# Fabstir/fabstir-vectordb

Measured on AMD Instinct MI355X. Metric: k-NN queries/sec at recall@10>=0.95, 1Mx384 f32, higher is better.
Workload: dtype f32

## Files before the change

### fabstir-vectordb_amd/csrc/fvdb_hip.cpp

```cpp
#include "fvdb_internal.h"

#include <unistd.h>

#include <algorithm>
#include <atomic>
#include <cmath>
#include <condition_variable>
#include <mutex>
#include <cstdio>
#include <cstdlib>
#include <cstring>
#include <map>
#include <new>
#include <string>
#include <vector>

#include "common.h"
#include "kernels_misc.h"
#include "kernels_scan.h"
#include "kernels_coarse.h"
#include "kernels_mfma.h"
#include "kernels_mfma_wg.h"
#include "kernels_util.h"
#include "kernels_maint.h"
// ... 115 lines not shown
  SC_STATS = 4,
};
constexpr size_t kScalarsBytes = 64;

struct IvfScratch {
  std::mutex enq;
  bool pend_filter = false;
  bool pending_profile = false, pend_coarse = false, pend_fine = false, collecting = false;
  std::vector<DBuf*> bufs;
  struct Buf : DBuf {
    explicit Buf(IvfScratch* set) { set->bufs.push_back(this); }
  };
  Buf s_qnorm{this}, s_A{this};
  Buf s_qh{this}, s_qn2{this}, s_thr{this}, s_tA{this}, s_pa{this}, s_surv{this}, s_scnt{this}, s_fail{this}, s_mslots{this};
  Buf s_sdist{this}, s_probes2{this};
  Buf s_q{this}, s_cpart{this}, s_probes{this}, s_cnt{this}, s_fill{this}, s_eoff{this}, s_ioff{this}, s_entries{this};
  Buf s_part{this}, s_scalars{this}, s_ceoff{this}, s_cioff{this};
  Buf s_in{this}, s_slots{this}, s_ids{this}, s_clusters{this}, s_out_ids{this}, s_out_dist{this}, s_out_cnt{this}, s_cdist{this};
  hipEvent_t sev[EV_COUNT] = {};
  uint32_t* scalar(ScalWord w) const { return s_scalars.as<uint32_t>() + w; }
  void release_all() {
    for (DBuf* b : bufs) b->release();
    for (auto& e : sev) {
      if (e) (void)hipEventDestroy(e);
      e = nullptr;
    }
  }
};

struct fvdb_ivf : IvfScratch {
  static constexpr uint32_t kSlots = 16;
// ... 70 lines not shown
  static bool has(const char* name) { return getenv(name) != nullptr; }
  static int tiles(int m) { return m >= 4 ? 4 : (m >= 2 ? 2 : 1); }
  bool coarse_exact = has("FVDB_COARSE_EXACT");
  bool scan_exact = has("FVDB_SCAN_EXACT");
  uint32_t scan_wgs_per_cu = (uint32_t)num("FVDB_SCAN_WGS_PER_CU", 8);
  int segb = num("FVDB_SEGB", 0);
  bool no_shared_thr = has("FVDB_NO_SHARED_THR");
  int mfma_m = tiles(num("FVDB_MFMA_M", 2));
  int mfma_segb = num("FVDB_MFMA_SEGB", 0);
  uint32_t mfma_wgs_per_cu = (uint32_t)std::max(1, num("FVDB_MFMA_WGS_PER_CU", 2));
  bool mfma_groups_in_item = num("FVDB_MFMA_GROUPS_IN_ITEM", 0) != 0;
  bool mfma_wg = num("FVDB_MFMA_WG", 1) != 0;
  int mfma_wg_m = num("FVDB_MFMA_WG_M", 4) >= 4 ? 4 : 2;
  uint32_t mfma_wg_segb = (uint32_t)std::max(4, num("FVDB_MFMA_WG_SEGB", 16));
  uint32_t mfma_wg_per_cu = (uint32_t)std::max(1, num("FVDB_MFMA_WG_PER_CU", 2));
  int mfma_wg_tail_pct = num("FVDB_MFMA_WG_TAIL_PCT", 25);
  int mfma_wg_segb_tail = num("FVDB_MFMA_WG_SEGB_TAIL", 4);
  uint32_t mfma_cap_a = (uint32_t)std::max(1, num("FVDB_MFMA_CAP_A", 4));
  bool mfma_threshold_pass = has("FVDB_MFMA_THRESHOLD_PASS");
  uint32_t mfma_segb_a = (uint32_t)std::max(1, num("FVDB_MFMA_SEGB_A", 1));
  bool mfma_no_refine = has("FVDB_MFMA_NO_REFINE");
#ifdef FVDB_MFMA_STAMPS_BUILD
  int mfma_stamps = num("FVDB_MFMA_STAMPS", 0);
#endif
};
const IvfKnobs& ivf_knobs() {
  static const IvfKnobs knobs{};
  return knobs;
}

struct ScanLaunch {
// ... 192 lines not shown
  if (max_blocks >= 4096) return 16;
  if (pairs >= 4096) return 4;
  if (pairs >= 512) return 2;
  return 1;
}
uint32_t pick_segb(fvdb_ivf* ivf, uint32_t B, uint32_t nprobe) {
  const int forced = ivf_knobs().segb;
  return forced > 0 ? (uint32_t)forced : segb_for(ivf->max_list_blocks, B, nprobe);
}
uint64_t queries_per_gib(uint32_t max_blocks, uint32_t segb, uint32_t k, uint32_t np) {
  const uint64_t per_q = (uint64_t)np * std::max<uint32_t>(1, cdiv(max_blocks, segb)) * k * 8;
  return (1ull << 30) / std::max<uint64_t>(per_q, 1);
}

void launch_plan(fvdb_ivf* ivf, const Env& E, const uint32_t* probes, uint32_t n, uint32_t np, uint32_t segb, uint32_t Q,
                 unsigned long long* stats, uint32_t* rezero_cnt, uint32_t lsplit = 0xFFFFFFFFu, uint32_t segb_tail = 0) {
  fvdb_ctx* ctx = E.ctx;
  IvfScratch& S = *E.S;
  const uint32_t* list_off = ivf->t_off.as<uint32_t>();
  hipLaunchKernelGGL(plan_count_kernel, dim3(cdiv(n, 256)), dim3(256), 0, ctx->stream, probes, n, S.s_cnt.as<uint32_t>(),
                     list_off);
  hipLaunchKernelGGL(plan_scan_kernel, dim3(1), dim3(1024), 0, ctx->stream, S.s_cnt.as<uint32_t>(), list_off,
                     ivf->t_len.as<uint32_t>(), ivf->nlist, segb, Q, S.s_eoff.as<uint32_t>(), S.s_ioff.as<uint32_t>(),
                     S.s_fill.as<uint32_t>(), S.scalar(SC_FINE_ITEMS), S.scalar(SC_FINE_HEAD), stats, rezero_cnt, lsplit,
                     segb_tail);
  hipLaunchKernelGGL(plan_fill_kernel, dim3(cdiv(n, 256)), dim3(256), 0, ctx->stream, probes, n, np,
                     S.s_eoff.as<uint32_t>(), S.s_fill.as<uint32_t>(), S.s_entries.as<uint2>(), list_off);
}
inline unsigned long long* scan_stats(const IvfScratch& S) { return (unsigned long long*)S.scalar(SC_STATS); }

int plan_scratch(fvdb_ivf* ivf, const Env& E, uint32_t B, uint32_t np) {
  fvdb_ctx* ctx = E.ctx;
  IvfScratch& S = *E.S;
  const uint32_t nlist = ivf->nlist;
  HIPCHK(ctx, S.s_cnt.ensure((size_t)nlist * 4));
  HIPCHK(ctx, S.s_fill.ensure((size_t)nlist * 4));
  HIPCHK(ctx, S.s_eoff.ensure((size_t)(nlist + 1) * 4));
  HIPCHK(ctx, S.s_ioff.ensure((size_t)(nlist + 1) * 4));
  HIPCHK(ctx, S.s_entries.ensure((size_t)B * np * 8));
  return FVDB_OK;
// ... 29 lines not shown

constexpr uint32_t kMfmaSlack = 6;
constexpr uint32_t kMfmaCmax = 4096;

bool mfma_shape_ok(const fvdb_ivf* ivf, uint32_t B, uint32_t k, uint32_t np) {
  return ivf->dpad % 16 == 0 && k + kMfmaSlack <= 32 && np <= 256 && B >= 32 && B <= 16384;
}
inline bool half_rows(const fvdb_ivf* ivf) { return ivf->f16 || ivf->pool.half != nullptr; }
inline int x_rounded(const fvdb_ivf* ivf) { return ivf->f16 ? 0 : (ivf->pool.half ? 1 : 2); }

struct MfmaPlan {
  bool wg;
  int M;
  uint32_t Q, ka, cmax;
  uint32_t segb, segbA;
  uint32_t lsplit, segb_tail;
  uint32_t fsegb, fmaxsegs;
  uint64_t fpart;
  uint32_t grid, wg_grid, wg_lds;
  bool half_rows;
  int x_rounded;
};

int mfma_plan(fvdb_ivf* ivf, fvdb_ctx* ctx, const IvfKnobs& kn, uint32_t B, uint32_t k, uint32_t np, MfmaPlan* out) {
  MfmaPlan P{};
  P.half_rows = half_rows(ivf);
  P.x_rounded = x_rounded(ivf);
  int wgM = kn.mfma_wg_m;
  if (mfma_wg_lds_bytes(ivf->dpad, 16u * wgM) > 64u * 1024u) wgM = 2;
  P.wg = kn.mfma_wg && kn.mfma_m == 2 && P.half_rows && ivf->dpad % 128 == 0 &&
         mfma_wg_lds_bytes(ivf->dpad, 16u * wgM) <= 64u * 1024u;
  P.M = P.wg ? wgM : kn.mfma_m;
  P.Q = 16u * P.M;
  P.ka = k + kMfmaSlack;
  P.cmax = kMfmaCmax;
  P.segbA = kn.mfma_segb_a;
  P.segb = P.wg ? kn.mfma_wg_segb : (kn.mfma_segb > 0 ? (uint32_t)kn.mfma_segb : pick_segb(ivf, B, np));
  P.lsplit = 0xFFFFFFFFu;
  P.segb_tail = P.segb;
  if (P.wg && kn.mfma_wg_tail_pct > 0 && kn.mfma_wg_segb_tail > 0 && (uint32_t)kn.mfma_wg_segb_tail < P.segb) {
    P.lsplit = (uint32_t)((uint64_t)ivf->nlist * (uint32_t)(100 - std::min(kn.mfma_wg_tail_pct, 100)) / 100);
    P.segb_tail = (uint32_t)kn.mfma_wg_segb_tail;
  }
  P.fsegb = pick_segb(ivf, B, np);
  P.fmaxsegs = std::max<uint32_t>(1, cdiv(ivf->max_list_blocks, P.fsegb));
  P.fpart = (uint64_t)B * np * P.fmaxsegs * k;
  if (P.fpart >= (1ull << 32)) FAIL(ctx, FVDB_E_UNSUPPORTED, "batch too large for one launch (sub-batch it)");
  P.grid = (uint32_t)ctx->num_cus * kn.mfma_wgs_per_cu;
  P.wg_grid = (uint32_t)ctx->num_cus * kn.mfma_wg_per_cu;
  P.wg_lds = mfma_wg_lds_bytes(ivf->dpad, P.Q);
  *out = P;
  return FVDB_OK;
}

int mfma_scratch(fvdb_ivf* ivf, const Env& E, const MfmaPlan& P, uint32_t B, uint32_t np) {
  fvdb_ctx* ctx = E.ctx;
  IvfScratch& S = *E.S;
  HIPCHK(ctx, S.s_qh.ensure((size_t)(B + 1) * ivf->dpad * 2));
  HIPCHK(ctx, S.s_qn2.ensure((size_t)B * 4));
  HIPCHK(ctx, S.s_thr.ensure((size_t)B * 4));
  HIPCHK(ctx, S.s_tA.ensure((size_t)B * 4));
  HIPCHK(ctx, S.s_pa.ensure((size_t)B * 4));
  HIPCHK(ctx, S.s_mslots.ensure((size_t)B * 64 * 4));
  HIPCHK(ctx, S.s_surv.ensure((size_t)B * P.cmax * 8));
  HIPCHK(ctx, S.s_sdist.ensure((size_t)B * P.cmax * 4));
  HIPCHK(ctx, S.s_scnt.ensure((size_t)(B + 2) * 4));
  HIPCHK(ctx, S.s_fail.ensure((size_t)B * 4));
  HIPCHK(ctx, S.s_part.ensure((size_t)P.fpart * 8));
  int rc = plan_scratch(ivf, E, B, np);
  if (rc) return rc;
  HIPCHK(ctx, S.s_scalars.ensure(kScalarsBytes));
  return FVDB_OK;
}

void launch_prep_queries(fvdb_ivf* ivf, const Env& E, const float* qpad, uint32_t B) {
  IvfScratch& S = *E.S;
  hipLaunchKernelGGL(prep_queries_kernel, dim3(cdiv(B + 1, 4)), dim3(256), 0, E.ctx->stream, qpad, B, ivf->dpad,
                     (_Float16*)S.s_qh.p, S.s_qn2.as<float>(), S.s_cnt.as<uint32_t>(), ivf->nlist,
                     S.s_scnt.as<uint32_t>(), S.s_mslots.as<uint32_t>());
}

ThresholdArgs threshold_args(fvdb_ivf* ivf, const IvfScratch& S, const float* qpad, const uint32_t* probes, uint32_t B,
                             uint32_t k, uint32_t np, float* thr_out) {
  ThresholdArgs t{};
  t.rows = ivf->pool.half ? ivf->pool.half : ivf->pool.data;
  t.pool_valid = ivf->pool.valid;
  t.pool_norms = ivf->pool.norms;
// ... 35 lines not shown
  a.entries = (const u32x2*)S.s_entries.p;
  a.n_items = S.scalar(SC_FINE_ITEMS);
  a.head = S.scalar(SC_FINE_HEAD);
  a.qh = (const _Float16*)S.s_qh.p;
  a.zero_row = B;
  a.dpad = ivf->dpad;
  a.segb = P.segb;
  a.thr = E.given_thr ? E.given_thr : S.s_thr.as<float>();
  a.cmax = P.cmax;
  a.surv = (u32x2*)S.s_surv.p;
  a.sval = S.s_sdist.as<float>();
  a.scnt = S.s_scnt.as<uint32_t>();
  a.slots = S.s_mslots.as<uint32_t>();
  a.capA = ivf_knobs().mfma_cap_a;
  a.groups_in_item = ivf_knobs().mfma_groups_in_item ? 1u : 0u;
  a.lsplit = P.lsplit;
  a.segb_tail = P.segb_tail;
  return a;
}

using MfmaKernel = decltype(&scan_mfma_kernel<2, 1, 0>);
template <int M, int MODE>
MfmaKernel mfma_kernel_of(bool f16) {
  return f16 ? scan_mfma_kernel<M, 1, MODE> : scan_mfma_kernel<M, 0, MODE>;
}
template <int MODE>
void launch_mfma(fvdb_ctx* ctx, const MfmaScanArgs& a, const MfmaPlan& P) {
  const MfmaKernel kernel = P.M == 1   ? mfma_kernel_of<1, MODE>(P.half_rows)
                            : P.M == 2 ? mfma_kernel_of<2, MODE>(P.half_rows)
                                       : mfma_kernel_of<4, MODE>(P.half_rows);
  hipLaunchKernelGGL(kernel, dim3(P.grid), dim3(256), 0, ctx->stream, a);
}
// ... 26 lines not shown
  }
}

#ifdef FVDB_MFMA_STAMPS_BUILD
constexpr uint32_t kStampsCap = 32768;
int mfma_stamps_begin(fvdb_ivf* ivf, fvdb_ctx* ctx, const MfmaPlan& P, MfmaScanArgs* a) {
  const int stamps_env = ivf_knobs().mfma_stamps;
  const bool stamp_now = P.wg && stamps_env && ++ivf->mfma_stamps_launch >= stamps_env && ivf->mfma_stamps_launch < stamps_env + 3;
  if (!stamp_now) return FVDB_OK;
  HIPCHK(ctx, ivf->d_mfma_stamps.ensure((size_t)kStampsCap * 64));
  HIPCHK(ctx, hipMemsetAsync(ivf->d_mfma_stamps.p, 0, (size_t)kStampsCap * 64, ctx->stream));
  a->stamps = ivf->d_mfma_stamps.as<unsigned long long>();
  a->stamps_cap = kStampsCap;
  return FVDB_OK;
}
int mfma_stamps_report(fvdb_ivf* ivf, fvdb_ctx* ctx, MfmaScanArgs* a) {
  if (!a->stamps) return FVDB_OK;
  HIPCHK(ctx, hipStreamSynchronize(ctx->stream));
  std::vector<unsigned long long> h((size_t)kStampsCap * 8);
  HIPCHK(ctx, hipMemcpy(h.data(), a->stamps, h.size() * 8, hipMemcpyDeviceToHost));
  unsigned long long t_min = ~0ull, t_max = 0;
  size_t n = 0;
  for (size_t i = 0; i < kStampsCap; ++i)
    if (h[i * 8 + 3]) {
      t_min = std::min(t_min, h[i * 8]);
      t_max = std::max(t_max, h[i * 8 + 3]);
      ++n;
    }
  double s_loc = 0, s_tile = 0, s_comp = 0, s_steps = 0, s_blocks = 0;
  size_t per_xcd[16] = {0};
  std::vector<double> per_step;
  for (size_t i = 0; i < kStampsCap; ++i) {
    const unsigned long long* r = &h[i * 8];
    if (!r[3]) continue;
    const double steps = (double)((r[5] + 3) / 4) * (double)(ivf->dpad / 16);
    s_loc += (double)(r[1] - r[0]);
    s_tile += (double)(r[2] - r[1]);
    s_comp += (double)(r[3] - r[2]);
    s_steps += steps;
    s_blocks += (double)r[5];
    per_xcd[r[7] & 15]++;
    per_step.push_back((double)(r[3] - r[2]) / steps);
  }
  std::sort(per_step.begin(), per_step.end());
  const double tick = 0.01;
  fprintf(stderr,
          "[mfma stamps] launch %d: %zu items, %0.f blocks, span %.1f us | per item (wave 0): locate %.2f us, tile %.2f us, "
          "compute %.2f us | per 16-dim step: mean %.3f us, p10 %.3f, p50 %.3f, p90 %.3f | items per XCD",
          ivf->mfma_stamps_launch, n, s_blocks, (double)(t_max - t_min) * tick, s_loc / n * tick, s_tile / n * tick, s_comp / n * tick,
          s_comp / s_steps * tick, per_step.empty() ? 0.0 : per_step[per_step.size() / 10] * tick,
          per_step.empty() ? 0.0 : per_step[per_step.size() / 2] * tick,
          per_step.empty() ? 0.0 : per_step[per_step.size() * 9 / 10] * tick);
  for (int x = 0; x < 8; ++x) fprintf(stderr, " %zu", per_xcd[x]);
  unsigned long long last_start = 0;
  for (size_t i = 0; i < kStampsCap; ++i)
    if (h[i * 8 + 3]) last_start = std::max(last_start, h[i * 8]);
  fprintf(stderr, " | last item drawn at %.1f us\n", (double)(last_start - t_min) * tick);
  a->stamps = nullptr;
  return FVDB_OK;
}
#else
inline int mfma_stamps_begin(fvdb_ivf*, fvdb_ctx*, const MfmaPlan&, MfmaScanArgs*) { return FVDB_OK; }
inline int mfma_stamps_report(fvdb_ivf*, fvdb_ctx*, MfmaScanArgs*) { return FVDB_OK; }
#endif

int mfma_filter(fvdb_ivf* ivf, const Env& E, const MfmaPlan& P, const Batch& b, MfmaScanArgs* a) {
  fvdb_ctx* ctx = E.ctx;
  launch_plan(ivf, E, b.probes, b.B * b.np, b.np, P.segb, P.Q, scan_stats(*E.S), E.S->s_cnt.as<uint32_t>(), P.lsplit,
              P.segb_tail);
  mark(ivf, E, EV_FILTER_BEGIN);
  int rc = mfma_stamps_begin(ivf, ctx, P, a);
  if (rc) return rc;
  launch_filter(ctx, *a, P);
  rc = mfma_stamps_report(ivf, ctx, a);
  if (rc) return rc;
  mark(ivf, E, EV_FILTER_DONE);
  return FVDB_OK;
}

bool auto_backs_off(fvdb_ivf* ivf) {
  std::lock_guard<std::mutex> lk(ivf->mu);
  if (ivf->exact_batches_left > 0) {
    ivf->exact_batches_left -= 1;
    return true;
  }
  if (!(ivf->h_fb.p && ivf->mfma_q - ivf->q_seen >= 2048)) return false;
  const uint64_t fb_now = ((volatile uint32_t*)ivf->h_fb.p)[FB_SCAN];
  const uint64_t dq = ivf->mfma_q - ivf->q_seen, dfb = fb_now - ivf->fb_seen;
  ivf->q_seen = ivf->mfma_q;
// ... 15 lines not shown
    ivf->overflow_seen = now;
    ivf->overflow_q = ivf->mfma_q;
  }
  if (ivf->refine_batches_left == 0) return false;
  ivf->refine_batches_left -= 1;
  return true;
}

int mfma_refine(fvdb_ivf* ivf, const Env& E, const MfmaPlan& P, const Batch& b, const MfmaScanArgs& a) {
  fvdb_ctx* ctx = E.ctx;
  IvfScratch& S = *E.S;
  HIPCHK(ctx, S.s_probes2.ensure((size_t)b.B * b.np * 4));
  hipLaunchKernelGGL(refine_threshold_kernel, dim3(cdiv(b.B, 4)), dim3(256), 0, ctx->stream, S.s_sdist.as<float>(),
                     S.s_scnt.as<uint32_t>(), b.probes, S.s_qn2.as<float>(), ivf->d_xmax.as<uint32_t>(), b.B, b.np, P.ka, P.cmax,
                     ivf->dpad, P.x_rounded, S.s_thr.as<float>(), S.s_probes2.as<uint32_t>(), ivf->fb_word(FB_REFINED));
  launch_plan(ivf, E, S.s_probes2.as<uint32_t>(), b.B * b.np, b.np, P.segb, P.Q, nullptr, S.s_cnt.as<uint32_t>(), P.lsplit,
              P.segb_tail);
  launch_filter(ctx, a, P);
  return FVDB_OK;
}

VerifyArgs verify_args(fvdb_ivf* ivf, const Env& E, const MfmaPlan& P, const Batch& b) {
  const IvfScratch& S = *E.S;
  VerifyArgs v{};
  v.pool = ivf->pool.view();
  v.lists = list_table(ivf);
  v.probes = b.probes;
  v.glob_blocks = ivf->t_glob.as<uint32_t>();
  v.queries = b.qpad;
  v.qn = S.s_qn2.as<float>();
  v.xmax_bits = ivf->d_xmax.as<uint32_t>();
  v.thr = E.given_thr ? E.given_thr : S.s_thr.as<float>();
// ... 1688 lines not shown
```

### fabstir-vectordb_amd/csrc/kernels_mfma.h

```cpp
#pragma once
#include "score_rows.h"
#include "common.h"
#include "kernels_scan.h"

#pragma clang fp contract(off)

#ifndef FVDB_MFMA_WAVES
#define FVDB_MFMA_WAVES 2
#endif

namespace fvdb {

typedef _Float16 h8v __attribute__((ext_vector_type(8)));
typedef __fp16 fp16x2v __attribute__((ext_vector_type(2)));
typedef uint32_t u32x4v __attribute__((ext_vector_type(4)));
__device__ __forceinline__ uint32_t pk_rtz(float a, float b) {
  return __builtin_bit_cast(uint32_t, __builtin_amdgcn_cvt_pkrtz(a, b));
}
typedef float f32x16m __attribute__((ext_vector_type(16)));

constexpr float kHalfMax = 65504.0f;

__global__ void pool_row_norms_kernel(const float* __restrict__ src, uint32_t d, uint64_t n, int f16,
                                      const uint32_t* __restrict__ dst_slot, float* __restrict__ norms,
// ... 84 lines not shown
  const uint32_t* n_items;
  uint32_t* head;
  const _Float16* qh;
  uint32_t zero_row;
  uint32_t dpad, segb;
  const float* thr;
  uint32_t cmax;
  u32x2* surv;
  float* sval;
  uint32_t* scnt;
  uint32_t* slots;
  uint32_t capA;
  uint32_t groups_in_item;
  unsigned long long* stamps;
  uint32_t stamps_cap;
  uint32_t lsplit, segb_tail;
};

template <int ST>
struct RowChunk16 {
  float4 v[4];
  h8v h[2];
};
template <int ST>
__device__ __forceinline__ void load_a16(const void* __restrict__ pool_data, uint32_t blk, uint32_t d4, uint32_t c4,
                                         int lane, RowChunk16<ST>& r) {
  if (ST == 0) {
    const float4* xp = (const float4*)pool_data + ((size_t)blk * d4 + c4) * 64 + lane;
    r.v[0] = xp[0];
    r.v[1] = xp[64];
    r.v[2] = xp[128];
// ... 789 lines not shown
```

### fabstir-vectordb_amd/csrc/kernels_mfma_wg.h

```cpp
#pragma once
#include "kernels_mfma.h"

#ifndef FVDB_MFMA_WG_WAVES
#define FVDB_MFMA_WG_WAVES 2
#endif

namespace fvdb {

#ifndef FVDB_MFMA_WG_RING
#define FVDB_MFMA_WG_RING 8
#endif
constexpr int kWgRing = FVDB_MFMA_WG_RING;
__host__ __device__ inline uint32_t mfma_wg_qstride(uint32_t dpad) { return dpad * 2u + 16u; }
__host__ __device__ inline uint32_t mfma_wg_lds_bytes(uint32_t dpad, uint32_t Q) { return (Q + 1u) * mfma_wg_qstride(dpad) + 16u; }

template <int M>
__device__ __forceinline__ void mfma_item_wg(const MfmaScanArgs& a, const unsigned char* __restrict__ qt,
                                             const uint32_t qstride, const uint32_t b_begin, const uint32_t bw,
                                             const uint32_t b1, const uint32_t e0, const uint32_t ne, const uint32_t zero_row,
                                             const int lane) {
  constexpr int D = M >= 3 ? 4 : kWgRing;
  const int j = lane & 31, g = lane >> 5, qs = j & 15;
  const bool opnd = g == (j >> 4);
  bool hasq[M];
  float thr[M];
  uint32_t qidx[M], rnk[M], qoff[M];
#pragma unroll
  for (int m = 0; m < M; ++m) {
    const uint32_t qi = 16 * m + qs;
    const bool has = qi < ne;
    const u32x2 e = a.entries[e0 + (has ? qi : 0)];
    qidx[m] = e.x;
    rnk[m] = e.y;
    hasq[m] = has;
    qoff[m] = ((opnd && has) ? qi : zero_row) * qstride;
// ... 38 lines not shown
    }
  };
#pragma unroll
  for (int u = 0; u < D - 1; ++u) issue_row(ring[u]);
  read_q(0, qf0[0], qf1[0]);
  uint32_t b = bw, cc = 0;
  for (uint32_t s = 0; s < total; s += D) {
    if (cc + D == n) load_block_norms(a, cload(a.list_blocks + b_begin + b), rowbase, bn);
#pragma unroll
    for (int u = 0; u < D; ++u) {
      issue_row(ring[(u + D - 1) & (D - 1)]);
      const uint32_t cn = cc + u + 1;
      read_q(cn >= n ? cn - n : cn, qf0[(u + 1) & 1], qf1[(u + 1) & 1]);
      h8v a0, a1;
      operands_a16<1>(ring[u], a0, a1);
#pragma unroll
      for (int m = 0; m < M; ++m) {
        acc[m] = __builtin_amdgcn_mfma_f32_32x32x16_f16(a0, qf0[u & 1][m], acc[m], 0, 0, 0);
        acc[m] = __builtin_amdgcn_mfma_f32_32x32x16_f16(a1, qf1[u & 1][m], acc[m], 0, 0, 0);
      }
    }
    cc += D;
    if (cc == n) {
      cc = 0;
      block_done(b);
      b += 4;
    }
  }
}

template <int QM>
__global__ __launch_bounds__(256, FVDB_MFMA_WG_WAVES) void scan_mfma_wg_kernel(const MfmaScanArgs a) {
  constexpr uint32_t Q = 16u * QM;
  extern __shared__ __attribute__((aligned(16))) unsigned char wg_lds[];
  const int lane = threadIdx.x & 63, w = threadIdx.x >> 6;
  const uint32_t qstride = mfma_wg_qstride(a.dpad);
  uint32_t* s_item = (uint32_t*)(wg_lds + (Q + 1u) * qstride);
  for (uint32_t i = threadIdx.x; i < qstride / 4; i += 256) ((uint32_t*)(wg_lds + Q * qstride))[i] = 0u;
  const uint32_t n_items = cload(a.n_items);
  const uint32_t ppr = a.dpad >> 3;
  for (;;) {
    __syncthreads();
    if (threadIdx.x == 0) *s_item = atomicAdd(a.head, 1u);
    __syncthreads();
    const uint32_t item = rfl(*s_item);
    if (item >= n_items) return;
#ifdef FVDB_MFMA_STAMPS_BUILD
    const unsigned long long t_drawn = wall_clock64();
#endif
    uint32_t lo = 0, hi = a.nlist;
    while (hi - lo > 1) {
      const uint32_t mid = (lo + hi) >> 1;
      if (cload(a.item_off + mid) <= item) lo = mid; else hi = mid;
    }
    const uint32_t L = lo;
    const uint32_t e_begin = cload(a.entry_off + L);
    const uint32_t cnt = cload(a.entry_off + L + 1) - e_begin;
    const uint32_t ngroups = (cnt + Q - 1u) / Q;
    const uint32_t local = item - cload(a.item_off + L);
    const uint32_t seg = local / ngroups, g = local - seg * ngroups;
    const uint32_t b_begin = cload(a.list_off + L);
    const uint32_t nblk = cload(a.list_off + L + 1) - b_begin;
    const uint32_t sb = L >= a.lsplit ? a.segb_tail : a.segb;
    const uint32_t b0 = seg * sb;
    const uint32_t b1 = min(b0 + sb, nblk);
    const uint32_t e0 = e_begin + g * Q;
    const uint32_t ne = min(Q, cnt - g * Q);
#ifdef FVDB_MFMA_STAMPS_BUILD
    const unsigned long long t_located = wall_clock64();
#endif
    const uint32_t pieces = ne * ppr;
    for (uint32_t p0 = threadIdx.x; p0 < pieces; p0 += 1024u) {
      h8v v[4];
      uint32_t dst[4];
#pragma unroll
      for (int t = 0; t < 4; ++t) {
        const uint32_t p = p0 + 256u * t;
        const bool in = p < pieces;
        const uint32_t qi = in ? p / ppr : 0u, c = in ? p - qi * ppr : 0u;
        const uint32_t qrow = a.entries[e0 + qi].x;
        v[t] = *(const h8v*)(a.qh + (size_t)qrow * a.dpad + 8u * c);
        dst[t] = in ? qi * qstride + 16u * c : 0xFFFFFFFFu;
      }
#pragma unroll
      for (int t = 0; t < 4; ++t)
        if (dst[t] != 0xFFFFFFFFu) *(h8v*)(wg_lds + dst[t]) = v[t];
    }
    __syncthreads();
#ifdef FVDB_MFMA_STAMPS_BUILD
    const unsigned long long t_tile = wall_clock64();
#endif
    if (ne <= 16)
      mfma_item_wg<1>(a, wg_lds, qstride, b_begin, b0 + (uint32_t)w, b1, e0, ne, Q, lane);
    else if (QM == 2 || ne <= 32)
      mfma_item_wg<2>(a, wg_lds, qstride, b_begin, b0 + (uint32_t)w, b1, e0, ne, Q, lane);
    else if (ne <= 48)
      mfma_item_wg<(QM >= 4 ? 3 : 2)>(a, wg_lds, qstride, b_begin, b0 + (uint32_t)w, b1, e0, ne, Q, lane);
    else
      mfma_item_wg<(QM >= 4 ? 4 : 2)>(a, wg_lds, qstride, b_begin, b0 + (uint32_t)w, b1, e0, ne, Q, lane);
#ifdef FVDB_MFMA_STAMPS_BUILD
    if (a.stamps && threadIdx.x == 0 && item < a.stamps_cap) {
      unsigned long long* r = a.stamps + (size_t)item * 8;
      r[0] = t_drawn;
      r[1] = t_located;
      r[2] = t_tile;
      r[3] = wall_clock64();
      r[4] = item;
      r[5] = b1 - b0;
      r[6] = ne;
      r[7] = __builtin_amdgcn_s_getreg((3 << 11) | 20);
    }
#endif
  }
}

}
```

### fabstir-vectordb_amd/csrc/kernels_scan.h

```cpp
#pragma once
#include "common.h"

#pragma clang fp contract(off)

namespace fvdb {

#if defined(__HIP_DEVICE_COMPILE__)
#define FVDB_CONST_AS __attribute__((address_space(4)))
#else
#define FVDB_CONST_AS
#endif
typedef float f32x4 __attribute__((ext_vector_type(4)));
typedef float f32x16_n __attribute__((ext_vector_type(16)));
typedef f32x16_n f32x16;
typedef uint32_t u32x2 __attribute__((ext_vector_type(2)));

template <typename T>
__device__ __forceinline__ T cload(const T* p) {
  return *(const FVDB_CONST_AS T*)(uintptr_t)p;
}

__device__ __forceinline__ f32x16_n cload16(const float* p) {
  typedef f32x16_n __attribute__((aligned(16))) f32x16_a;
  return *(const FVDB_CONST_AS f32x16_a*)(uintptr_t)p;
// ... 368 lines not shown
      out_dist[o] = have ? __uint_as_float(khi) : __uint_as_float(0x7F800000u);
    }
  }
  if (lane == 0 && out_counts) out_counts[q] = count;
}

__global__ void plan_count_kernel(const uint32_t* __restrict__ probes, uint32_t n, uint32_t* __restrict__ cnt,
                                  const uint32_t* __restrict__ list_off = nullptr) {
  const uint32_t i = blockIdx.x * blockDim.x + threadIdx.x;
  if (i < n) {
    const uint32_t L = probes[i];
    if (L != kInf32 && (!list_off || list_off[L + 1] != list_off[L])) atomicAdd(cnt + L, 1u);
  }
}

__global__ __launch_bounds__(1024) void plan_scan_kernel(const uint32_t* __restrict__ cnt,
                                                         const uint32_t* __restrict__ list_off,
                                                         const uint32_t* __restrict__ list_len, uint32_t nlist,
                                                         uint32_t segb, uint32_t Q, uint32_t* __restrict__ entry_off,
                                                         uint32_t* __restrict__ item_off, uint32_t* __restrict__ fill,
                                                         uint32_t* __restrict__ n_items, uint32_t* __restrict__ head,
                                                         unsigned long long* __restrict__ stats,
                                                         uint32_t* __restrict__ rezero_cnt = nullptr,
                                                         uint32_t lsplit = 0xFFFFFFFFu, uint32_t segb_tail = 0) {
  __shared__ uint32_t s_e[1024], s_i[1024];
  __shared__ uint32_t carry_e, carry_i;
  __shared__ unsigned long long s_rows, s_touch;
  const uint32_t t = threadIdx.x;
  if (t == 0) {
    carry_e = carry_i = 0;
    s_rows = s_touch = 0;
  }
  __syncthreads();
  for (uint32_t base = 0; base < nlist; base += 1024) {
    const uint32_t L = base + t;
    uint32_t c = 0, it = 0;
    if (L < nlist) {
      c = cnt[L];
      if (rezero_cnt) rezero_cnt[L] = 0;
      const uint32_t nblk = list_off[L + 1] - list_off[L];
      const uint32_t sb = L >= lsplit ? segb_tail : segb;
      const uint32_t nseg = (nblk + sb - 1) / sb;
      it = (c == 0 || nblk == 0) ? 0u : nseg * ((c + Q - 1) / Q);
      fill[L] = 0;
      if (c) {
        atomicAdd(&s_rows, (unsigned long long)c * list_len[L]);
        atomicAdd(&s_touch, (unsigned long long)list_len[L]);
      }
    }
    s_e[t] = c;
    s_i[t] = it;
    __syncthreads();
    for (uint32_t ofs = 1; ofs < 1024; ofs <<= 1) {
      uint32_t ve = 0, vi = 0;
      if (t >= ofs) {
        ve = s_e[t - ofs];
        vi = s_i[t - ofs];
// ... 11 lines not shown
    if (t == 1023) {
      carry_e += s_e[1023];
      carry_i += s_i[1023];
    }
    __syncthreads();
  }
  if (t == 0) {
    entry_off[nlist] = carry_e;
    item_off[nlist] = carry_i;
    *n_items = carry_i;
    *head = 0;
    if (stats) {
      stats[0] = s_rows;
      stats[1] = carry_i;
      stats[2] = s_touch;
    }
  }
}

__global__ void plan_fill_kernel(const uint32_t* __restrict__ probes, uint32_t n, uint32_t nprobe,
                                 const uint32_t* __restrict__ entry_off, uint32_t* __restrict__ fill,
                                 uint2* __restrict__ entries, const uint32_t* __restrict__ list_off = nullptr) {
  const uint32_t i = blockIdx.x * blockDim.x + threadIdx.x;
  if (i < n) {
    const uint32_t L = probes[i];
    if (L != kInf32 && (!list_off || list_off[L + 1] != list_off[L])) {
      const uint32_t p = atomicAdd(fill + L, 1u);
      entries[entry_off[L] + p] = make_uint2(i / nprobe, i % nprobe);
    }
  }
// ... 26 lines not shown
```

Before: 1.660 million.

## Precompute cost-sorted item records for MFMA workgroup scan and prefetch next item

The plan kernel now emits an explicit per-item record array (block range, entry offset, query count), ordered by estimated cost in descending order. Only the cheapest items, up to a tail percentage of total cost, are split into smaller segments. The workgroup scan kernel reads these records instead of binary-searching item offsets. One wave prefetches the next record and its query row ids into LDS, which removes the per-item locate latency and a barrier and gives longest-first load balancing. The trade-off is extra serial work in the single-block plan kernel, an extra scratch buffer, and a changed default tail percentage.

```diff
diff --git a/fabstir-vectordb_amd/csrc/fvdb_hip.cpp b/fabstir-vectordb_amd/csrc/fvdb_hip.cpp
--- a/fabstir-vectordb_amd/csrc/fvdb_hip.cpp
+++ b/fabstir-vectordb_amd/csrc/fvdb_hip.cpp
@@ -153,7 +153,7 @@
   Buf s_qnorm{this}, s_A{this};
   Buf s_qh{this}, s_qn2{this}, s_thr{this}, s_tA{this}, s_pa{this}, s_surv{this}, s_scnt{this}, s_fail{this}, s_mslots{this};
   Buf s_sdist{this}, s_probes2{this};
-  Buf s_q{this}, s_cpart{this}, s_probes{this}, s_cnt{this}, s_fill{this}, s_eoff{this}, s_ioff{this}, s_entries{this};
+  Buf s_q{this}, s_cpart{this}, s_probes{this}, s_cnt{this}, s_fill{this}, s_eoff{this}, s_ioff{this}, s_entries{this}, s_recs{this};
   Buf s_part{this}, s_scalars{this}, s_ceoff{this}, s_cioff{this};
   Buf s_in{this}, s_slots{this}, s_ids{this}, s_clusters{this}, s_out_ids{this}, s_out_dist{this}, s_out_cnt{this}, s_cdist{this};
   hipEvent_t sev[EV_COUNT] = {};
@@ -254,7 +254,7 @@
   int mfma_wg_m = num("FVDB_MFMA_WG_M", 4) >= 4 ? 4 : 2;
   uint32_t mfma_wg_segb = (uint32_t)std::max(4, num("FVDB_MFMA_WG_SEGB", 16));
   uint32_t mfma_wg_per_cu = (uint32_t)std::max(1, num("FVDB_MFMA_WG_PER_CU", 2));
-  int mfma_wg_tail_pct = num("FVDB_MFMA_WG_TAIL_PCT", 25);
+  int mfma_wg_tail_pct = std::clamp(num("FVDB_MFMA_WG_TAIL_PCT", 12), 0, 100);
   int mfma_wg_segb_tail = num("FVDB_MFMA_WG_SEGB_TAIL", 4);
   uint32_t mfma_cap_a = (uint32_t)std::max(1, num("FVDB_MFMA_CAP_A", 4));
   bool mfma_threshold_pass = has("FVDB_MFMA_THRESHOLD_PASS");
@@ -477,7 +477,7 @@
 }
 
 void launch_plan(fvdb_ivf* ivf, const Env& E, const uint32_t* probes, uint32_t n, uint32_t np, uint32_t segb, uint32_t Q,
-                 unsigned long long* stats, uint32_t* rezero_cnt, uint32_t lsplit = 0xFFFFFFFFu, uint32_t segb_tail = 0) {
+                 unsigned long long* stats, uint32_t* rezero_cnt, const ItemPlan items = ItemPlan{nullptr, 0, 0, 0}) {
   fvdb_ctx* ctx = E.ctx;
   IvfScratch& S = *E.S;
   const uint32_t* list_off = ivf->t_off.as<uint32_t>();
@@ -485,8 +485,7 @@
                      list_off);
   hipLaunchKernelGGL(plan_scan_kernel, dim3(1), dim3(1024), 0, ctx->stream, S.s_cnt.as<uint32_t>(), list_off,
                      ivf->t_len.as<uint32_t>(), ivf->nlist, segb, Q, S.s_eoff.as<uint32_t>(), S.s_ioff.as<uint32_t>(),
-                     S.s_fill.as<uint32_t>(), S.scalar(SC_FINE_ITEMS), S.scalar(SC_FINE_HEAD), stats, rezero_cnt, lsplit,
-                     segb_tail);
+                     S.s_fill.as<uint32_t>(), S.scalar(SC_FINE_ITEMS), S.scalar(SC_FINE_HEAD), stats, rezero_cnt, items);
   hipLaunchKernelGGL(plan_fill_kernel, dim3(cdiv(n, 256)), dim3(256), 0, ctx->stream, probes, n, np,
                      S.s_eoff.as<uint32_t>(), S.s_fill.as<uint32_t>(), S.s_entries.as<uint2>(), list_off);
 }
@@ -546,7 +545,8 @@
   int M;
   uint32_t Q, ka, cmax;
   uint32_t segb, segbA;
-  uint32_t lsplit, segb_tail;
+  uint32_t segb_tail, tail_pct;
+  uint64_t item_cap;
   uint32_t fsegb, fmaxsegs;
   uint64_t fpart;
   uint32_t grid, wg_grid, wg_lds;
@@ -568,12 +568,17 @@
   P.cmax = kMfmaCmax;
   P.segbA = kn.mfma_segb_a;
   P.segb = P.wg ? kn.mfma_wg_segb : (kn.mfma_segb > 0 ? (uint32_t)kn.mfma_segb : pick_segb(ivf, B, np));
-  P.lsplit = 0xFFFFFFFFu;
   P.segb_tail = P.segb;
+  P.tail_pct = 0;
   if (P.wg && kn.mfma_wg_tail_pct > 0 && kn.mfma_wg_segb_tail > 0 && (uint32_t)kn.mfma_wg_segb_tail < P.segb) {
-    P.lsplit = (uint32_t)((uint64_t)ivf->nlist * (uint32_t)(100 - std::min(kn.mfma_wg_tail_pct, 100)) / 100);
     P.segb_tail = (uint32_t)kn.mfma_wg_segb_tail;
-  }
+    P.tail_pct = (uint32_t)kn.mfma_wg_tail_pct;
+  }
+  const uint64_t pairs = (uint64_t)B * np;
+  P.item_cap = P.wg ? (pairs / P.Q + std::min<uint64_t>(ivf->nlist, pairs)) *
+                          std::max<uint32_t>(1, cdiv(ivf->max_list_blocks, P.segb)) * cdiv(P.segb, P.segb_tail)
+                    : 0;
+  if (P.item_cap >= (1ull << 32) - 1) FAIL(ctx, FVDB_E_UNSUPPORTED, "batch too large for one launch (sub-batch it)");
   P.fsegb = pick_segb(ivf, B, np);
   P.fmaxsegs = std::max<uint32_t>(1, cdiv(ivf->max_list_blocks, P.fsegb));
   P.fpart = (uint64_t)B * np * P.fmaxsegs * k;
@@ -599,10 +604,14 @@
   HIPCHK(ctx, S.s_scnt.ensure((size_t)(B + 2) * 4));
   HIPCHK(ctx, S.s_fail.ensure((size_t)B * 4));
   HIPCHK(ctx, S.s_part.ensure((size_t)P.fpart * 8));
+  if (P.wg) HIPCHK(ctx, S.s_recs.ensure((size_t)(P.item_cap + 1) * 16));
   int rc = plan_scratch(ivf, E, B, np);
   if (rc) return rc;
   HIPCHK(ctx, S.s_scalars.ensure(kScalarsBytes));
   return FVDB_OK;
+}
+inline ItemPlan item_plan(const IvfScratch& S, const MfmaPlan& P) {
+  return P.wg ? ItemPlan{(uint4*)S.s_recs.p, (uint32_t)P.item_cap, P.segb_tail, P.tail_pct} : ItemPlan{nullptr, 0, 0, 0};
 }
 
 void launch_prep_queries(fvdb_ivf* ivf, const Env& E, const float* qpad, uint32_t B) {
@@ -668,8 +677,7 @@
   a.slots = S.s_mslots.as<uint32_t>();
   a.capA = ivf_knobs().mfma_cap_a;
   a.groups_in_item = ivf_knobs().mfma_groups_in_item ? 1u : 0u;
-  a.lsplit = P.lsplit;
-  a.segb_tail = P.segb_tail;
+  a.recs = P.wg ? (const u32x4v*)S.s_recs.p : nullptr;
   return a;
 }
 
@@ -726,21 +734,28 @@
   a->stamps_cap = kStampsCap;
   return FVDB_OK;
 }
-int mfma_stamps_report(fvdb_ivf* ivf, fvdb_ctx* ctx, MfmaScanArgs* a) {
+int mfma_stamps_report(fvdb_ivf* ivf, fvdb_ctx* ctx, const MfmaPlan& P, MfmaScanArgs* a) {
   if (!a->stamps) return FVDB_OK;
   HIPCHK(ctx, hipStreamSynchronize(ctx->stream));
   std::vector<unsigned long long> h((size_t)kStampsCap * 8);
   HIPCHK(ctx, hipMemcpy(h.data(), a->stamps, h.size() * 8, hipMemcpyDeviceToHost));
-  unsigned long long t_min = ~0ull, t_max = 0;
+  unsigned long long t_min = ~0ull, t_max = 0, last_start = 0;
   size_t n = 0;
-  for (size_t i = 0; i < kStampsCap; ++i)
-    if (h[i * 8 + 3]) {
-      t_min = std::min(t_min, h[i * 8]);
-      t_max = std::max(t_max, h[i * 8 + 3]);
-      ++n;
-    }
-  double s_loc = 0, s_tile = 0, s_comp = 0, s_steps = 0, s_blocks = 0;
-  size_t per_xcd[16] = {0};
+  std::vector<unsigned long long> wg_end(P.wg_grid, 0);
+  for (size_t i = 0; i < kStampsCap; ++i) {
+    const unsigned long long* r = &h[i * 8];
+    if (!r[3]) continue;
+    t_min = std::min(t_min, r[0]);
+    t_max = std::max(t_max, r[3]);
+    last_start = std::max(last_start, r[0]);
+    const size_t wg = (size_t)(r[7] >> 8);
+    if (wg < wg_end.size()) wg_end[wg] = std::max(wg_end[wg], r[3]);
+    ++n;
+  }
+  if (!n) return FVDB_OK;
+  double s_loc = 0, s_tile = 0, s_pro = 0, s_stream = 0, s_steps = 0, s_blocks = 0;
+  double m_time[5] = {0}, m_blocks[5] = {0};
+  size_t per_xcd[16] = {0}, m_items[5] = {0};
   std::vector<double> per_step;
   for (size_t i = 0; i < kStampsCap; ++i) {
     const unsigned long long* r = &h[i * 8];
@@ -748,43 +763,71 @@
     const double steps = (double)((r[5] + 3) / 4) * (double)(ivf->dpad / 16);
     s_loc += (double)(r[1] - r[0]);
     s_tile += (double)(r[2] - r[1]);
-    s_comp += (double)(r[3] - r[2]);
+    s_pro += (double)(r[4] - r[2]);
+    s_stream += (double)(r[3] - r[4]);
     s_steps += steps;
     s_blocks += (double)r[5];
     per_xcd[r[7] & 15]++;
     per_step.push_back((double)(r[3] - r[2]) / steps);
+    const size_t m = std::min<size_t>(4, (r[6] + 15) / 16);
+    m_items[m]++;
+    m_blocks[m] += (double)((r[5] + 3) / 4);
+    m_time[m] += (double)(r[3] - r[2]);
   }
   std::sort(per_step.begin(), per_step.end());
   const double tick = 0.01;
+  const double span = (double)(t_max - t_min);
+  size_t wgs = 0;
+  unsigned long long first_exit = ~0ull;
+  for (unsigned long long e : wg_end)
+    if (e) {
+      ++wgs;
+      first_exit = std::min(first_exit, e);
+    }
+  const double wg_time = span * (double)std::max<size_t>(wgs, 1);
   fprintf(stderr,
-          "[mfma stamps] launch %d: %zu items, %0.f blocks, span %.1f us | per item (wave 0): locate %.2f us, tile %.2f us, "
-          "compute %.2f us | per 16-dim step: mean %.3f us, p10 %.3f, p50 %.3f, p90 %.3f | items per XCD",
-          ivf->mfma_stamps_launch, n, s_blocks, (double)(t_max - t_min) * tick, s_loc / n * tick, s_tile / n * tick, s_comp / n * tick,
-          s_comp / s_steps * tick, per_step.empty() ? 0.0 : per_step[per_step.size() / 10] * tick,
-          per_step.empty() ? 0.0 : per_step[per_step.size() / 2] * tick,
-          per_step.empty() ? 0.0 : per_step[per_step.size() * 9 / 10] * tick);
+          "[mfma stamps] launch %d: %zu items, %0.f blocks, %zu workgroups, span %.1f us | per item (wave 0): locate %.2f us, "
+          "tile %.2f us, first rows %.2f us, stream %.2f us | share of workgroup-time: locate %.3f, tile %.3f, first rows %.3f, "
+          "stream %.3f, between items and idle %.3f | per 16-dim step: mean %.3f us, p10 %.3f, p50 %.3f, p90 %.3f | items per XCD",
+          ivf->mfma_stamps_launch, n, s_blocks, wgs, span * tick, s_loc / n * tick, s_tile / n * tick, s_pro / n * tick,
+          s_stream / n * tick, s_loc / wg_time, s_tile / wg_time, s_pro / wg_time, s_stream / wg_time,
+          1.0 - (s_loc + s_tile + s_pro + s_stream) / wg_time, (s_pro + s_stream) / s_steps * tick,
+          per_step[per_step.size() / 10] * tick, per_step[per_step.size() / 2] * tick, per_step[per_step.size() * 9 / 10] * tick);
   for (int x = 0; x < 8; ++x) fprintf(stderr, " %zu", per_xcd[x]);
-  unsigned long long last_start = 0;
-  for (size_t i = 0; i < kStampsCap; ++i)
-    if (h[i * 8 + 3]) last_start = std::max(last_start, h[i * 8]);
-  fprintf(stderr, " | last item drawn at %.1f us\n", (double)(last_start - t_min) * tick);
+  fprintf(stderr, " | us per block round of a wave by query tiles:");
+  for (int m = 1; m <= 4; ++m)
+    fprintf(stderr, " M%d %.2f (%zu items)", m, m_blocks[m] > 0 ? m_time[m] / m_blocks[m] * tick : 0.0, m_items[m]);
+  fprintf(stderr, " | last item drawn at %.1f us (%.3f of the launch), first workgroup done at %.3f\n",
+          (double)(last_start - t_min) * tick, (double)(last_start - t_min) / span, (double)(first_exit - t_min) / span);
+  if (const char* dump = getenv("FVDB_MFMA_STAMPS_DUMP")) {
+    if (FILE* f = fopen(dump, "w")) {
+      fprintf(f, "item,drawn,located,tile,first_rows,done,blocks,queries,xcd,workgroup\n");
+      for (size_t i = 0; i < kStampsCap; ++i) {
+        const unsigned long long* r = &h[i * 8];
+        if (r[3])
+          fprintf(f, "%zu,%llu,%llu,%llu,%llu,%llu,%llu,%llu,%llu,%llu\n", i, r[0] - t_min, r[1] - t_min, r[2] - t_min,
+                  r[4] - t_min, r[3] - t_min, r[5], r[6], r[7] & 15, r[7] >> 8);
+      }
+      fclose(f);
+    }
+  }
   a->stamps = nullptr;
   return FVDB_OK;
 }
 #else
 inline int mfma_stamps_begin(fvdb_ivf*, fvdb_ctx*, const MfmaPlan&, MfmaScanArgs*) { return FVDB_OK; }
-inline int mfma_stamps_report(fvdb_ivf*, fvdb_ctx*, MfmaScanArgs*) { return FVDB_OK; }
+inline int mfma_stamps_report(fvdb_ivf*, fvdb_ctx*, const MfmaPlan&, MfmaScanArgs*) { return FVDB_OK; }
 #endif
 
 int mfma_filter(fvdb_ivf* ivf, const Env& E, const MfmaPlan& P, const Batch& b, MfmaScanArgs* a) {
   fvdb_ctx* ctx = E.ctx;
-  launch_plan(ivf, E, b.probes, b.B * b.np, b.np, P.segb, P.Q, scan_stats(*E.S), E.S->s_cnt.as<uint32_t>(), P.lsplit,
-              P.segb_tail);
+  launch_plan(ivf, E, b.probes, b.B * b.np, b.np, P.segb, P.Q, scan_stats(*E.S), E.S->s_cnt.as<uint32_t>(),
+              item_plan(*E.S, P));
   mark(ivf, E, EV_FILTER_BEGIN);
   int rc = mfma_stamps_begin(ivf, ctx, P, a);
   if (rc) return rc;
   launch_filter(ctx, *a, P);
-  rc = mfma_stamps_report(ivf, ctx, a);
+  rc = mfma_stamps_report(ivf, ctx, P, a);
   if (rc) return rc;
   mark(ivf, E, EV_FILTER_DONE);
   return FVDB_OK;
@@ -830,8 +873,8 @@
   hipLaunchKernelGGL(refine_threshold_kernel, dim3(cdiv(b.B, 4)), dim3(256), 0, ctx->stream, S.s_sdist.as<float>(),
                      S.s_scnt.as<uint32_t>(), b.probes, S.s_qn2.as<float>(), ivf->d_xmax.as<uint32_t>(), b.B, b.np, P.ka, P.cmax,
                      ivf->dpad, P.x_rounded, S.s_thr.as<float>(), S.s_probes2.as<uint32_t>(), ivf->fb_word(FB_REFINED));
-  launch_plan(ivf, E, S.s_probes2.as<uint32_t>(), b.B * b.np, b.np, P.segb, P.Q, nullptr, S.s_cnt.as<uint32_t>(), P.lsplit,
-              P.segb_tail);
+  launch_plan(ivf, E, S.s_probes2.as<uint32_t>(), b.B * b.np, b.np, P.segb, P.Q, nullptr, S.s_cnt.as<uint32_t>(),
+              item_plan(S, P));
   launch_filter(ctx, a, P);
   return FVDB_OK;
 }
diff --git a/fabstir-vectordb_amd/csrc/kernels_mfma.h b/fabstir-vectordb_amd/csrc/kernels_mfma.h
--- a/fabstir-vectordb_amd/csrc/kernels_mfma.h
+++ b/fabstir-vectordb_amd/csrc/kernels_mfma.h
@@ -122,7 +122,7 @@
   uint32_t groups_in_item;
   unsigned long long* stamps;
   uint32_t stamps_cap;
-  uint32_t lsplit, segb_tail;
+  const u32x4v* recs;
 };
 
 template <int ST>
diff --git a/fabstir-vectordb_amd/csrc/kernels_mfma_wg.h b/fabstir-vectordb_amd/csrc/kernels_mfma_wg.h
--- a/fabstir-vectordb_amd/csrc/kernels_mfma_wg.h
+++ b/fabstir-vectordb_amd/csrc/kernels_mfma_wg.h
@@ -12,13 +12,13 @@
 #endif
 constexpr int kWgRing = FVDB_MFMA_WG_RING;
 __host__ __device__ inline uint32_t mfma_wg_qstride(uint32_t dpad) { return dpad * 2u + 16u; }
-__host__ __device__ inline uint32_t mfma_wg_lds_bytes(uint32_t dpad, uint32_t Q) { return (Q + 1u) * mfma_wg_qstride(dpad) + 16u; }
+__host__ __device__ inline uint32_t mfma_wg_lds_bytes(uint32_t dpad, uint32_t Q) { return (Q + 1u) * mfma_wg_qstride(dpad) + 32u + 256u; }
 
 template <int M>
 __device__ __forceinline__ void mfma_item_wg(const MfmaScanArgs& a, const unsigned char* __restrict__ qt,
                                              const uint32_t qstride, const uint32_t b_begin, const uint32_t bw,
                                              const uint32_t b1, const uint32_t e0, const uint32_t ne, const uint32_t zero_row,
-                                             const int lane) {
+                                             const int lane, unsigned long long* t_first = nullptr) {
   constexpr int D = M >= 3 ? 4 : kWgRing;
   const int j = lane & 31, g = lane >> 5, qs = j & 15;
   const bool opnd = g == (j >> 4);
@@ -87,6 +87,12 @@
       read_q(cn >= n ? cn - n : cn, qf0[(u + 1) & 1], qf1[(u + 1) & 1]);
       h8v a0, a1;
       operands_a16<1>(ring[u], a0, a1);
+#ifdef FVDB_MFMA_STAMPS_BUILD
+      if (t_first && s == 0 && u == 0) {
+        asm volatile("" ::"v"(a0));
+        *t_first = wall_clock64();
+      }
+#endif
 #pragma unroll
       for (int m = 0; m < M; ++m) {
         acc[m] = __builtin_amdgcn_mfma_f32_32x32x16_f16(a0, qf0[u & 1][m], acc[m], 0, 0, 0);
@@ -108,38 +114,34 @@
   extern __shared__ __attribute__((aligned(16))) unsigned char wg_lds[];
   const int lane = threadIdx.x & 63, w = threadIdx.x >> 6;
   const uint32_t qstride = mfma_wg_qstride(a.dpad);
-  uint32_t* s_item = (uint32_t*)(wg_lds + (Q + 1u) * qstride);
+  uint32_t* s_next = (uint32_t*)(wg_lds + (Q + 1u) * qstride);
+  uint32_t* s_qrow = s_next + 8;
   for (uint32_t i = threadIdx.x; i < qstride / 4; i += 256) ((uint32_t*)(wg_lds + Q * qstride))[i] = 0u;
   const uint32_t n_items = cload(a.n_items);
   const uint32_t ppr = a.dpad >> 3;
+  auto draw = [&]() {
+    uint32_t t = 0;
+    if (lane == 0) t = atomicAdd(a.head, 1u);
+    t = rfl(t);
+    const u32x4v r = cload(a.recs + min(t, n_items));
+    const uint32_t e0 = rfl(r.z), ne = rfl(r.w) & 255u;
+    s_qrow[lane] = a.entries[e0 + min((uint32_t)lane, ne ? ne - 1u : 0u)].x;
+    if (lane == 0) {
+      *(u32x4v*)s_next = r;
+      s_next[4] = t;
+    }
+  };
+  if (w == 3) draw();
+#ifdef FVDB_MFMA_STAMPS_BUILD
+  unsigned long long t_drawn = wall_clock64();
+#endif
   for (;;) {
     __syncthreads();
-    if (threadIdx.x == 0) *s_item = atomicAdd(a.head, 1u);
-    __syncthreads();
-    const uint32_t item = rfl(*s_item);
-    if (item >= n_items) return;
+    const u32x4v rec = *(const u32x4v*)s_next;
+    const uint32_t b0 = rfl(rec.y), b_begin = rfl(rec.x) - b0, e0 = rfl(rec.z), ne = rfl(rec.w) & 255u, nb = rfl(rec.w) >> 8;
+    if (nb == 0) return;
 #ifdef FVDB_MFMA_STAMPS_BUILD
-    const unsigned long long t_drawn = wall_clock64();
-#endif
-    uint32_t lo = 0, hi = a.nlist;
-    while (hi - lo > 1) {
-      const uint32_t mid = (lo + hi) >> 1;
-      if (cload(a.item_off + mid) <= item) lo = mid; else hi = mid;
-    }
-    const uint32_t L = lo;
-    const uint32_t e_begin = cload(a.entry_off + L);
-    const uint32_t cnt = cload(a.entry_off + L + 1) - e_begin;
-    const uint32_t ngroups = (cnt + Q - 1u) / Q;
-    const uint32_t local = item - cload(a.item_off + L);
-    const uint32_t seg = local / ngroups, g = local - seg * ngroups;
-    const uint32_t b_begin = cload(a.list_off + L);
-    const uint32_t nblk = cload(a.list_off + L + 1) - b_begin;
-    const uint32_t sb = L >= a.lsplit ? a.segb_tail : a.segb;
-    const uint32_t b0 = seg * sb;
-    const uint32_t b1 = min(b0 + sb, nblk);
-    const uint32_t e0 = e_begin + g * Q;
-    const uint32_t ne = min(Q, cnt - g * Q);
-#ifdef FVDB_MFMA_STAMPS_BUILD
+    const uint32_t item = rfl(s_next[4]);
     const unsigned long long t_located = wall_clock64();
 #endif
     const uint32_t pieces = ne * ppr;
@@ -151,7 +153,7 @@
         const uint32_t p = p0 + 256u * t;
         const bool in = p < pieces;
         const uint32_t qi = in ? p / ppr : 0u, c = in ? p - qi * ppr : 0u;
-        const uint32_t qrow = a.entries[e0 + qi].x;
+        const uint32_t qrow = s_qrow[qi];
         v[t] = *(const h8v*)(a.qh + (size_t)qrow * a.dpad + 8u * c);
         dst[t] = in ? qi * qstride + 16u * c : 0xFFFFFFFFu;
       }
@@ -162,15 +164,20 @@
     __syncthreads();
 #ifdef FVDB_MFMA_STAMPS_BUILD
     const unsigned long long t_tile = wall_clock64();
+    unsigned long long t_first = t_tile;
+#define FVDB_WG_T_FIRST , &t_first
+#else
+#define FVDB_WG_T_FIRST
 #endif
+    const uint32_t b1 = b0 + nb;
     if (ne <= 16)
-      mfma_item_wg<1>(a, wg_lds, qstride, b_begin, b0 + (uint32_t)w, b1, e0, ne, Q, lane);
+      mfma_item_wg<1>(a, wg_lds, qstride, b_begin, b0 + (uint32_t)w, b1, e0, ne, Q, lane FVDB_WG_T_FIRST);
     else if (QM == 2 || ne <= 32)
-      mfma_item_wg<2>(a, wg_lds, qstride, b_begin, b0 + (uint32_t)w, b1, e0, ne, Q, lane);
+      mfma_item_wg<2>(a, wg_lds, qstride, b_begin, b0 + (uint32_t)w, b1, e0, ne, Q, lane FVDB_WG_T_FIRST);
     else if (ne <= 48)
-      mfma_item_wg<(QM >= 4 ? 3 : 2)>(a, wg_lds, qstride, b_begin, b0 + (uint32_t)w, b1, e0, ne, Q, lane);
+      mfma_item_wg<(QM >= 4 ? 3 : 2)>(a, wg_lds, qstride, b_begin, b0 + (uint32_t)w, b1, e0, ne, Q, lane FVDB_WG_T_FIRST);
     else
-      mfma_item_wg<(QM >= 4 ? 4 : 2)>(a, wg_lds, qstride, b_begin, b0 + (uint32_t)w, b1, e0, ne, Q, lane);
+      mfma_item_wg<(QM >= 4 ? 4 : 2)>(a, wg_lds, qstride, b_begin, b0 + (uint32_t)w, b1, e0, ne, Q, lane FVDB_WG_T_FIRST);
 #ifdef FVDB_MFMA_STAMPS_BUILD
     if (a.stamps && threadIdx.x == 0 && item < a.stamps_cap) {
       unsigned long long* r = a.stamps + (size_t)item * 8;
@@ -178,12 +185,14 @@
       r[1] = t_located;
       r[2] = t_tile;
       r[3] = wall_clock64();
-      r[4] = item;
-      r[5] = b1 - b0;
+      r[4] = t_first;
+      r[5] = nb;
       r[6] = ne;
-      r[7] = __builtin_amdgcn_s_getreg((3 << 11) | 20);
+      r[7] = (__builtin_amdgcn_s_getreg((3 << 11) | 20) & 15u) | (blockIdx.x << 8);
     }
+    t_drawn = wall_clock64();
 #endif
+    if (w == 3) draw();
   }
 }
 
diff --git a/fabstir-vectordb_amd/csrc/kernels_scan.h b/fabstir-vectordb_amd/csrc/kernels_scan.h
--- a/fabstir-vectordb_amd/csrc/kernels_scan.h
+++ b/fabstir-vectordb_amd/csrc/kernels_scan.h
@@ -406,6 +406,95 @@
   }
 }
 
+struct ItemPlan {
+  uint4* recs;
+  uint32_t cap;
+  uint32_t segb_tail;
+  uint32_t tail_pct;
+};
+constexpr uint32_t kItemKeys = 256;
+__device__ __forceinline__ uint32_t item_cost(uint32_t nb, uint32_t tiles) { return ((nb + 3u) >> 2) * (18u + tiles); }
+__device__ __forceinline__ uint32_t item_key(uint32_t nb, uint32_t tiles) { return min(item_cost(nb, tiles), kItemKeys - 1u); }
+
+template <typename F>
+__device__ __forceinline__ void plan_list_runs(uint32_t c, uint32_t nblk, uint32_t segb, uint32_t Q, uint32_t segb_tail,
+                                               uint32_t kcut, F&& f) {
+  if (c == 0 || nblk == 0) return;
+  const uint32_t ngroups = (c + Q - 1) / Q;
+  const uint32_t last_tiles = (c - (ngroups - 1) * Q + 15u) / 16u;
+  for (uint32_t b0 = 0; b0 < nblk; b0 += segb) {
+    const uint32_t nb = min(segb, nblk - b0);
+    const uint32_t tiles = ngroups > 1 ? Q / 16u : last_tiles;
+    if (item_cost(nb, tiles) <= kcut && nb > segb_tail) {
+      for (uint32_t s0 = 0; s0 < nb; s0 += segb_tail) f(b0 + s0, min(segb_tail, nb - s0), 0u, ngroups, tiles);
+    } else {
+      f(b0, nb, 0u, ngroups, tiles);
+    }
+  }
+}
+
+__device__ __forceinline__ void block_scan256(uint32_t* s, uint32_t t) {
+  for (uint32_t ofs = 1; ofs < 256; ofs <<= 1) {
+    const uint32_t v = (t < 256 && t >= ofs) ? s[t - ofs] : 0u;
+    __syncthreads();
+    if (t < 256) s[t] += v;
+    __syncthreads();
+  }
+}
+
+__device__ __forceinline__ uint32_t plan_item_records(const uint32_t* entry_off,
+                                                      const uint32_t* __restrict__ list_off, uint32_t nlist, uint32_t segb,
+                                                      uint32_t Q, const ItemPlan ip, uint32_t* s_a, uint32_t* s_b) {
+  const uint32_t t = threadIdx.x;
+  uint32_t* hist = s_a;
+  uint32_t* pos = s_a + 256;
+  __shared__ uint32_t s_kcut;
+  auto each_list = [&](uint32_t kcut, auto&& f) {
+    for (uint32_t L = t; L < nlist; L += 1024) {
+      const uint32_t e_begin = entry_off[L], c = entry_off[L + 1] - e_begin;
+      const uint32_t b_begin = list_off[L], nblk = list_off[L + 1] - b_begin;
+      plan_list_runs(c, nblk, segb, Q, ip.segb_tail, kcut,
+                     [&](uint32_t b0, uint32_t nb, uint32_t g0, uint32_t ng, uint32_t tiles) {
+                       f(e_begin, c, b_begin, b0, nb, g0, ng, tiles);
+                     });
+    }
+  };
+  auto count = [&](uint32_t kcut) {
+    if (t < 256) hist[t] = 0;
+    __syncthreads();
+    each_list(kcut, [&](uint32_t, uint32_t, uint32_t, uint32_t, uint32_t nb, uint32_t, uint32_t ng, uint32_t tiles) {
+      atomicAdd(&hist[item_key(nb, tiles)], ng);
+    });
+    __syncthreads();
+  };
+  count(0);
+  uint32_t kcut = 0;
+  if (ip.tail_pct > 0 && ip.segb_tail < segb) {
+    if (t < 256) s_b[t] = t * hist[t];
+    if (t == 0) s_kcut = 0;
+    __syncthreads();
+    block_scan256(s_b, t);
+    if (t < 256 && (unsigned long long)s_b[t] * 100ull <= (unsigned long long)s_b[255] * ip.tail_pct) atomicMax(&s_kcut, t);
+    __syncthreads();
+    kcut = s_kcut;
+    if (kcut > 0) count(kcut);
+  }
+  if (t < 256) s_b[t] = hist[255 - t];
+  __syncthreads();
+  block_scan256(s_b, t);
+  if (t < 256) pos[255 - t] = s_b[t] - hist[255 - t];
+  __syncthreads();
+  const uint32_t total = min(s_b[255], ip.cap);
+  each_list(kcut, [&](uint32_t e_begin, uint32_t c, uint32_t b_begin, uint32_t b0, uint32_t nb, uint32_t g0, uint32_t ng,
+                      uint32_t tiles) {
+    const uint32_t p = atomicAdd(&pos[item_key(nb, tiles)], ng);
+    for (uint32_t g = 0; g < ng; ++g)
+      if (p + g < ip.cap) ip.recs[p + g] = make_uint4(b_begin + b0, b0, e_begin + (g0 + g) * Q, min(Q, c - (g0 + g) * Q) | (nb << 8));
+  });
+  if (t == 0) ip.recs[total] = make_uint4(0u, 0u, 0u, 0u);
+  return total;
+}
+
 __global__ __launch_bounds__(1024) void plan_scan_kernel(const uint32_t* __restrict__ cnt,
                                                          const uint32_t* __restrict__ list_off,
                                                          const uint32_t* __restrict__ list_len, uint32_t nlist,
@@ -414,7 +503,7 @@
                                                          uint32_t* __restrict__ n_items, uint32_t* __restrict__ head,
                                                          unsigned long long* __restrict__ stats,
                                                          uint32_t* __restrict__ rezero_cnt = nullptr,
-                                                         uint32_t lsplit = 0xFFFFFFFFu, uint32_t segb_tail = 0) {
+                                                         const ItemPlan ip = ItemPlan{nullptr, 0, 0, 0}) {
   __shared__ uint32_t s_e[1024], s_i[1024];
   __shared__ uint32_t carry_e, carry_i;
   __shared__ unsigned long long s_rows, s_touch;
@@ -431,8 +520,7 @@
       c = cnt[L];
       if (rezero_cnt) rezero_cnt[L] = 0;
       const uint32_t nblk = list_off[L + 1] - list_off[L];
-      const uint32_t sb = L >= lsplit ? segb_tail : segb;
-      const uint32_t nseg = (nblk + sb - 1) / sb;
+      const uint32_t nseg = (nblk + segb - 1) / segb;
       it = (c == 0 || nblk == 0) ? 0u : nseg * ((c + Q - 1) / Q);
       fill[L] = 0;
       if (c) {
@@ -474,6 +562,14 @@
       stats[0] = s_rows;
       stats[1] = carry_i;
       stats[2] = s_touch;
+    }
+  }
+  if (ip.recs) {
+    __syncthreads();
+    const uint32_t n_recs = plan_item_records(entry_off, list_off, nlist, segb, Q, ip, s_e, s_i);
+    if (t == 0) {
+      *n_items = n_recs;
+      if (stats) stats[1] = n_recs;
     }
   }
 }
```

After: 1.693 million, median of 5. Within noise of the previous version (+2.0%).
